# SaeedRahmani/MPC_for_AV_at_Intersection

Hardware: AMD Instinct MI355X
Metric: MPC timesteps/sec (whole node), N=20 horizon, 8-agent intersection, batch=4096 (higher is better)
Workload: dtype f64

## Files before the change

### mpc_for_av_at_intersection_amd/csrc/mpcx_common.h

```cpp
#pragma once
#include <hip/hip_runtime.h>
#include <stdint.h>
#include "mpcx.h"
#include "mpcx_qp_consts.h"
#include <vector>

struct mpcx_ctx {
    int device = 0;
    hipStream_t stream = nullptr;
    mpcx_mpc_params mpc = {};
    bool have_mpc = false;
    int32_t *ticket = nullptr;
    int n_cu = 0;
    double *pred = nullptr;
    size_t pred_cap = 0;
    hipGraphExec_t loop_exec = nullptr;
    unsigned char loop_key[1192] = {};
    const mpcx_qp_tuning *tune = nullptr;
    int32_t tune_rows = 0;
    const int32_t *order_hint = nullptr;
    const int32_t *order_now = nullptr, *order_prev = nullptr;
    int32_t *prev_cut = nullptr;
    size_t prev_cut_cap = 0;
    int32_t *order = nullptr;
    size_t order_cap = 0;
    int32_t *bins = nullptr;
    size_t bins_cap = 0;
    bool bins_clean = false;
    hipStream_t side = nullptr;
    hipEvent_t ev_fork = nullptr, ev_join = nullptr;
    double *cs = nullptr;
    size_t cs_cap = 0;
    void *multi = nullptr;
    size_t multi_cap = 0;
    int qp_solver = 0;
    int lin_passes = 1;
    bool prof_qp = false;
    std::vector<hipEvent_t> prof_ev;
    std::vector<hipEvent_t> prof_free;
    unsigned long long *stats = nullptr;
    size_t stats_slots = 0;
    void *comm = nullptr;
    int comm_world = 1, comm_rank = 0;
    double *xchg = nullptr;
    size_t xchg_cap = 0;
    double *admit_tab = nullptr;
    size_t admit_tab_cap = 0;
    char err[256] = {};
};

struct mpcx_interaction_extras {
    const double *pack_state = nullptr, *pack_applied = nullptr;
    const int32_t *ego_row = nullptr, *actor_row = nullptr;
    int32_t n_ego = 0, n_actors = 0;
    int32_t *prev_save = nullptr;
    const int32_t *key_prev = nullptr;
    int32_t *near = nullptr;
    const int32_t *bin_hint = nullptr;
    const int32_t *done = nullptr;
    const int32_t *absent = nullptr;
    const int32_t *prec = nullptr;
    double *stand = nullptr;
};
struct mpcx_window_extras {
    bool scatter = false;
    const int32_t *near = nullptr, *tidx = nullptr;
    bool rollout_forked = false;
    const int32_t *stop_idx = nullptr;
    double v_ref = 0.0;
    int32_t *len_seen = nullptr;
    const int32_t *done = nullptr;
    int32_t *queue_len = nullptr;
};
struct mpcx_qp_order {
    bool ready = false;
    const int32_t *hint = nullptr, *now = nullptr, *prev = nullptr;
    const int32_t *queue_len = nullptr;
};
struct mpcx_plant_extras {
    const int32_t *stats_iters = nullptr;
    bool reset_bins = false;
    const int32_t *done = nullptr;
};
int32_t mpcx_interaction_enqueue(mpcx_ctx *ctx, const mpcx_interaction_params *ip, int32_t P, const double *state, const double *path_xyyaw,
                               const double *path_cs, const int32_t *path_off, const int32_t *path_len, const int32_t *prev_cut_len,
                               int32_t n_obs_pool, const double *obs6, const int32_t *obs_off, const int32_t *obs_cnt, const int32_t *obs_skip,
                               int32_t *traj_idx, int32_t *hit_idx, double *hit_xy, int32_t *cut_len, const mpcx_interaction_extras &x);
int32_t mpcx_window_enqueue(mpcx_ctx *ctx, int32_t B, const double *state, const double *u_warm, const double *path_xyyaw, const double *path_v,
                          const int32_t *path_off, const int32_t *path_len, double dl, int32_t *target_ind, const double *ov, int64_t ov_stride,
                          double *xref, uint8_t *reaches_end, double *xbar, const mpcx_window_extras &x);
int32_t mpcx_qp_enqueue(mpcx_ctx *ctx, int32_t B, const double *x0, const double *xref, const double *xbar, const uint8_t *reaches_end,
                      const double *u_warm, double *x_out, double *u_out, int32_t *status, int32_t *iters, double *kkt, const mpcx_qp_order &ord);
int32_t mpcx_plant_enqueue(mpcx_ctx *ctx, int32_t B, double *state, double *u, const int32_t *status, double *applied, const mpcx_plant_extras &x);

int32_t mpcx_fail(mpcx_ctx *ctx, int32_t code, const char *fmt, ...);
int32_t mpcx_check_launch(mpcx_ctx *ctx, const char *what);
int32_t mpcx_grow(mpcx_ctx *ctx, void **p, size_t *cap_bytes, size_t need_bytes, const char *what);
int32_t mpcx_ensure_pred(mpcx_ctx *ctx, size_t need_doubles);
int32_t mpcx_rollout_fork(mpcx_ctx *ctx, int32_t B, const double *state, const double *u_warm, double *xbar, const int32_t *done = nullptr);
int32_t mpcx_traffic_validate(mpcx_ctx *ctx, int32_t n_actors, const mpcx_traffic_actor *actors, const double *tape, int64_t tape_rows,
                              const int32_t *pool_row, int32_t n_obs_pool);
int32_t mpcx_traffic_enqueue(mpcx_ctx *ctx, int32_t n_actors, const mpcx_traffic_actor *actors, double *actor_state, const double *tape,
                             int64_t tape_rows, const int32_t *pool_row, int32_t n_obs_pool, double *obs6);
bool mpcx_record_absent(const mpcx_run_log *log);
int32_t mpcx_record_validate(mpcx_ctx *ctx, const mpcx_run_log *log, const int32_t *obs_skip);
int32_t mpcx_record_enqueue(mpcx_ctx *ctx, const mpcx_interaction_params *ip, int32_t P, const double *state, const double *applied,
                            const double *x_sol, const double *path_xyyaw, const int32_t *path_off, const int32_t *path_len,
                            const int32_t *target_ind, const int32_t *cut_len, const int32_t *traj_idx, const int32_t *hit_idx,
                            const int32_t *status, const int32_t *iters, int32_t n_obs_pool, const double *obs6, const int32_t *obs_off,
                            const int32_t *obs_cnt, const int32_t *obs_skip, const mpcx_run_log *log,
                            const int32_t *goal_len = nullptr,
                            const int32_t *done = nullptr,
                            const int32_t *absent = nullptr);
bool mpcx_retire_absent(const mpcx_retire *r);
int32_t mpcx_retire_validate(mpcx_ctx *ctx, const mpcx_retire *r, int32_t P);
int32_t mpcx_retire_enqueue(mpcx_ctx *ctx, int32_t P, const double *state, double *applied, const double *path_xyyaw, const int32_t *path_off,
                            const int32_t *path_len, const int32_t *target_ind, const int32_t *goal_len, const mpcx_retire *r,
                            const mpcx_scene *scene = nullptr, const int32_t *own_row = nullptr);
bool mpcx_scene_absent(const mpcx_scene *s);
int32_t mpcx_scene_validate(mpcx_ctx *ctx, const mpcx_scene *s, const mpcx_retire *retire, int32_t exchange, size_t pool_rows, const int32_t *obs_skip);
bool mpcx_admit_absent(const mpcx_admit *a);
int32_t mpcx_admit_validate(mpcx_ctx *ctx, const mpcx_admit *a, const mpcx_retire *retire, const mpcx_scene *scene, int32_t exchange);
int32_t mpcx_admit_prepare(mpcx_ctx *ctx, size_t n_rows);
int32_t mpcx_admit_enqueue(mpcx_ctx *ctx, const mpcx_interaction_params *ip, int32_t P, const double *state, const int32_t *obs_off,
                           const int32_t *obs_cnt, const int32_t *obs_skip, int32_t *done, int32_t n_obs_pool, int32_t *absent,
                           int32_t n_actors, const mpcx_traffic_actor *actors, const double *actor_state, const double *tape,
                           int64_t tape_rows, const int32_t *actor_row, const mpcx_admit *admit);
bool mpcx_respawn_absent(const mpcx_respawn *s);
int32_t mpcx_respawn_validate(mpcx_ctx *ctx, const mpcx_respawn *s, const mpcx_admit *admit);
int32_t mpcx_respawn_enqueue(mpcx_ctx *ctx, int32_t P, double *state, double *applied, double *u_sol, int32_t *traj_idx, int32_t *target_ind,
                             int32_t *cut_len, int32_t *iters, int32_t *prev_len , const int32_t *obs_skip, int32_t n_obs_pool,
                             const mpcx_run_log *log , const mpcx_retire *retire, const mpcx_admit *admit,
                             const mpcx_respawn *respawn);
bool mpcx_routes_absent(const mpcx_routes *s);
int32_t mpcx_routes_validate(mpcx_ctx *ctx, const mpcx_routes *s, const mpcx_respawn *respawn, const int32_t *path_off, const int32_t *path_len,
                             int32_t max_len );
int32_t mpcx_route_enqueue(mpcx_ctx *ctx, int32_t P, double *state, double *applied, double *u_sol, int32_t *traj_idx, int32_t *target_ind,
                           int32_t *cut_len, int32_t *iters, int32_t *prev_len , const int32_t *obs_skip, int32_t n_obs_pool,
                           const mpcx_run_log *log , const mpcx_retire *retire, const mpcx_admit *admit,
                           const mpcx_respawn *respawn, const mpcx_routes *routes);
bool mpcx_precedence_absent(const mpcx_precedence *s);
int32_t mpcx_precedence_validate(mpcx_ctx *ctx, const mpcx_precedence *s, const mpcx_scene *scene, const mpcx_admit *admit);
int32_t mpcx_precedence_enqueue(mpcx_ctx *ctx, int32_t P, const int32_t *obs_off, const int32_t *obs_skip, const mpcx_admit *admit,
                                const mpcx_precedence *precedence);
bool mpcx_signals_absent(const mpcx_signals *s);
int32_t mpcx_signals_validate(mpcx_ctx *ctx, const mpcx_signals *s, int32_t exchange);
int32_t mpcx_signal_enqueue(mpcx_ctx *ctx, int32_t P, double dl, const double *state, const int32_t *path_off, const int32_t *path_len,
                            const int32_t *traj_idx, int32_t *cut_len, const int32_t *done , const mpcx_signals *signals);
int32_t mpcx_ensure_ticket(mpcx_ctx *ctx);
#define MPCX_JUMP_BONUS 11
#define MPCX_ORDER_BINS 64
#define MPCX_TICKET_WORDS 8
#define MPCX_TICKET_QUEUE_LEN 6
#define MPCX_ORDER_COPIES 16
namespace mpcx {
__device__ __forceinline__ int order_key_of(int hint, bool moved) {
    int k = hint < 0 ? 0 : hint;
    if (moved) k += MPCX_JUMP_BONUS;
    return k < MPCX_ORDER_BINS ? k : MPCX_ORDER_BINS - 1;
}
}
int32_t mpcx_ensure_order(mpcx_ctx *ctx, size_t B);
int32_t mpcx_qp_build_order(mpcx_ctx *ctx, int32_t B, const int32_t *hint, const int32_t *now, const int32_t *prev, hipStream_t st);

namespace mpcx {

constexpr int WAVE = 64;

struct QpArgs {
    mpcx_mpc_params p;
    int B;
    int32_t *ticket;
    int has_warm;
    const double *x0, *xref, *xbar, *u_warm;
    const uint8_t *re;
    double *x_out, *u_out, *kkt;
    int32_t *status, *iters;
    const mpcx_qp_tuning *tune;
    int has_tune;
    const int32_t *order;
    int has_order;
    int defer_fail;
    int32_t *fail_list, *fail_count;
    const int32_t *queue_len;
    int has_queue_len;
};

void launch_qp_stage(const QpArgs &a, hipStream_t st, int n_cu);
int qp_stage_grid(int B, int n_cu);

__device__ __forceinline__ double rdlane(double v, int l) {
    int lo = __double2loint(v), hi = __double2hiint(v);
    lo = __builtin_amdgcn_readlane(lo, l);
    hi = __builtin_amdgcn_readlane(hi, l);
    return __hiloint2double(hi, lo);
}
__device__ __forceinline__ double frcp(double d) {
    double r = __builtin_amdgcn_rcp(d);
    r = fma(fma(-d, r, 1.0), r, r);
    r = fma(fma(-d, r, 1.0), r, r);
    return r;
}

template <int CTRL, int ROW_MASK = 0xF>
__device__ __forceinline__ double dpp_mov(double old, double src) {
    int lo = __builtin_amdgcn_update_dpp(__double2loint(old), __double2loint(src), CTRL, ROW_MASK, 0xF, false);
    int hi = __builtin_amdgcn_update_dpp(__double2hiint(old), __double2hiint(src), CTRL, ROW_MASK, 0xF, false);
    return __hiloint2double(hi, lo);
}
__device__ __forceinline__ double lane_next(double v, double fill = 0.0) { return dpp_mov<0x130>(fill, v); }
__device__ __forceinline__ double lane_prev(double v, double fill = 0.0) { return dpp_mov<0x138>(fill, v); }

__device__ __forceinline__ double scan_up32(double v) {
    v += dpp_mov<0x111>(0.0, v);
    v += dpp_mov<0x112>(0.0, v);
    v += dpp_mov<0x114>(0.0, v);
    v += dpp_mov<0x118>(0.0, v);
    v += dpp_mov<0x142, 0xA>(0.0, v);
    return v;
}
__device__ __forceinline__ double scan_down32(double v, int lane) {
    v += dpp_mov<0x101>(0.0, v);
    v += dpp_mov<0x102>(0.0, v);
    v += dpp_mov<0x104>(0.0, v);
    v += dpp_mov<0x108>(0.0, v);
    const double r1 = rdlane(v, 16);
    return v + ((lane < 16) ? r1 : 0.0);
}
__device__ __forceinline__ double wave_sum_dpp(double v) {
    v += dpp_mov<0x111>(0.0, v);
    v += dpp_mov<0x112>(0.0, v);
    v += dpp_mov<0x114>(0.0, v);
    v += dpp_mov<0x118>(0.0, v);
    return (rdlane(v, 15) + rdlane(v, 31)) + (rdlane(v, 47) + rdlane(v, 63));
}
__device__ __forceinline__ double wave_max_dpp(double v) {
    v = fmax(v, dpp_mov<0x111>(v, v));
    v = fmax(v, dpp_mov<0x112>(v, v));
    v = fmax(v, dpp_mov<0x114>(v, v));
    v = fmax(v, dpp_mov<0x118>(v, v));
    return fmax(fmax(rdlane(v, 15), rdlane(v, 31)), fmax(rdlane(v, 47), rdlane(v, 63)));
}
__device__ __forceinline__ double frcp1(double d) {
    double r = __builtin_amdgcn_rcp(d);
    return fma(fma(-d, r, 1.0), r, r);
}

__device__ __forceinline__ void wave_argmin(double &d, int &i) {
#pragma unroll
    for (int s = 32; s >= 1; s >>= 1) {
        double od = __shfl_xor(d, s, WAVE);
        int oi = __shfl_xor(i, s, WAVE);
        bool take = (od < d) || (od == d && oi < i);
        d = take ? od : d;
        i = take ? oi : i;
    }
}

template <typename T>
__device__ __forceinline__ T wave_min_i(T v) {
#pragma unroll
    for (int s = 32; s >= 1; s >>= 1) { T o = __shfl_xor(v, s, WAVE); v = o < v ? o : v; }
    return v;
}

__device__ __forceinline__ void disc_centre(double px, double py, double c, double s, double cx, double cy, double &ex, double &ey) {
    ex = __dadd_rn(__dadd_rn(__dmul_rn(c, cx), -__dmul_rn(s, cy)), px);
    ey = __dadd_rn(__dadd_rn(__dmul_rn(s, cx), __dmul_rn(c, cy)), py);
}

struct Top3 {
    double d0 = INFINITY, d1 = INFINITY, d2 = INFINITY, s2 = INFINITY, s1 = INFINITY, s0 = INFINITY;
    int i0 = 0x7fffffff, i1 = 0x7fffffff, i2 = 0x7fffffff;
    __device__ __forceinline__ void offer(double px, double py, double x, double y, int i) {
        const double dx = __dadd_rn(px, -x), dy = __dadd_rn(py, -y);
        const double q = __dadd_rn(__dmul_rn(dx, dx), __dmul_rn(dy, dy));
        if (q < s2 || i2 == 0x7fffffff) {
            const double d = __dsqrt_rn(q);
            if (d < d2 || (d == d2 && i < i2)) {
                if (d < d1 || (d == d1 && i < i1)) {
                    d2 = d1; i2 = i1; s2 = s1;
                    if (d < d0 || (d == d0 && i < i0)) { d1 = d0; i1 = i0; s1 = s0; d0 = d; i0 = i; s0 = q; }
                    else { d1 = d; i1 = i; s1 = q; }
                } else { d2 = d; i2 = i; s2 = q; }
            }
        }
    }
    __device__ __forceinline__ void pop3(int (&bi)[3]) {
#pragma unroll
        for (int r = 0; r < 3; r++) {
            double d = d0; int ix = i0;
            wave_argmin(d, ix);
            bi[r] = ix;
            if (i0 == ix) { d0 = d1; i0 = i1; d1 = d2; i1 = i2; d2 = INFINITY; i2 = 0x7fffffff; }
        }
    }
};
__device__ __forceinline__ int three_nearest(const int (&bi)[3], int base) {
    if (abs(bi[1] - bi[2]) == 2) return bi[0] + base;
    if (abs(bi[0] - bi[1]) == 1) return max(bi[0], bi[1]) + base;
    return -1;
}

__device__ inline int nearest_index_in_direction(const double *path, int n, int start, double x, double y, int lane) {
    const int len = n - start;
    if (len <= 1) return start;
    if (len == 2) return start + 1;
    Top3 top;
    constexpr int DEPTH = 4;
    double bx[DEPTH], by[DEPTH];
#pragma unroll
    for (int k = 0; k < DEPTH; k++) {
        const int i = k * WAVE + lane;
        const double *q = path + 3 * (size_t)(start + (i < len ? i : 0));
        const double vx = q[0], vy = q[1];
        bx[k] = vx; by[k] = vy;
    }
    for (int i0 = 0; i0 < len; i0 += DEPTH * WAVE) {
        double nbx[DEPTH], nby[DEPTH];
#pragma unroll
        for (int k = 0; k < DEPTH; k++) {
            const int i = i0 + (DEPTH + k) * WAVE + lane;
            const double *q = path + 3 * (size_t)(start + (i < len ? i : 0));
            nbx[k] = q[0]; nby[k] = q[1];
        }
#pragma unroll
        for (int k = 0; k < DEPTH; k++) {
            const int i = i0 + k * WAVE + lane;
            if (i < len) top.offer(bx[k], by[k], x, y, i);
        }
#pragma unroll
        for (int k = 0; k < DEPTH; k++) { bx[k] = nbx[k]; by[k] = nby[k]; }
    }
    int bi[3];
#pragma unroll
    for (int r = 0; r < 3; r++) {
        double d = top.d0; int ix = top.i0;
        wave_argmin(d, ix);
        bi[r] = ix;
        if (top.i0 == ix) { top.d0 = top.d1; top.i0 = top.i1; top.d1 = top.d2; top.i1 = top.i2; top.d2 = INFINITY; top.i2 = 0x7fffffff; }
    }
    return three_nearest(bi, start);
}

}
```

### mpc_for_av_at_intersection_amd/csrc/mpcx_qp_quad.hip

```cpp
#include "mpcx_common.h"
#include "mpcx_qp_stage.h"

namespace mpcx {

typedef __attribute__((address_space(3))) double lds_double;

template <int LQ_, int SPL_, bool JERK_ = false>
struct GroupCx {
    static constexpr int LQ = LQ_, SPL = SPL_;
    static constexpr bool JERK = JERK_;
    static_assert(LQ == 8, "groups of 8 lanes");
    int q, lane;
    lds_double *sh;
    __device__ __forceinline__ double nxt(double v) const { return dpp_mov<0x101>(v, v); }
    __device__ __forceinline__ double prv(double v) const { return dpp_mov<0x111>(v, v); }
    __device__ __forceinline__ double gsum(double v) const {
        v += dpp_mov<0xB1>(v, v); v += dpp_mov<0x4E>(v, v);
        v += dpp_mov<0x141>(v, v);
        return v;
    }
    __device__ __forceinline__ double gmax(double v) const {
        v = fmax(v, dpp_mov<0xB1>(v, v)); v = fmax(v, dpp_mov<0x4E>(v, v));
        v = fmax(v, dpp_mov<0x141>(v, v));
        return v;
    }
    __device__ __forceinline__ double gmin(double v) const {
        v = fmin(v, dpp_mov<0xB1>(v, v)); v = fmin(v, dpp_mov<0x4E>(v, v));
        v = fmin(v, dpp_mov<0x141>(v, v));
        return v;
    }
    __device__ __forceinline__ bool gany(bool b) const {
        const unsigned long long m = __ballot(b);
        return ((m >> (lane & ~(LQ - 1))) & ((1ull << LQ) - 1ull)) != 0ull;
    }
    __device__ __forceinline__ bool any(bool b) const { return __ballot(b) != 0ull; }
    __device__ __forceinline__ int count(bool b) const { return __popcll(__ballot(b)); }
    __device__ __forceinline__ double rcp(double v) const { return frcp(v); }
    __device__ __forceinline__ double rcp_fast(double v) const { return frcp1(v); }
    __device__ __forceinline__ double rcp_seed(double v) const { return __builtin_amdgcn_rcp(v); }
    __device__ __forceinline__ void fence() const { asm volatile("" ::: "memory"); }
    __device__ __forceinline__ void stamp(int) const {}
    __device__ __forceinline__ double ld_s(int k) const { return sh[(0 * SPL * 8 + k) * 64 + lane]; }
    __device__ __forceinline__ double ld_l(int k) const { return sh[(1 * SPL * 8 + k) * 64 + lane]; }
    __device__ __forceinline__ double ld_k(int k) const { return sh[(2 * SPL * 8 + k) * 64 + lane]; }
    __device__ __forceinline__ void st_s(int k, double v) { sh[(0 * SPL * 8 + k) * 64 + lane] = v; }
    __device__ __forceinline__ void st_l(int k, double v) { sh[(1 * SPL * 8 + k) * 64 + lane] = v; }
    __device__ __forceinline__ void st_k(int k, double v) { sh[(2 * SPL * 8 + k) * 64 + lane] = v; }
    __device__ __forceinline__ double ld_w(int k) const { return sh[(3 * SPL * 8 + k) * 64 + lane]; }
    __device__ __forceinline__ void st_w(int k, double v) { sh[(3 * SPL * 8 + k) * 64 + lane] = v; }
};

constexpr int REFILL_GROUPS = 2;
template <int LQ, int SPL, bool TUNED>
struct QueueSrc {
    const QpArgs &a;
    __device__ __forceinline__ mpcx_mpc_params params() const { return a.p; }
    __device__ __forceinline__ mpcx_stage::Problem at(int b) const {
        const int T = a.p.T, W = T + 1;
        return mpcx_stage::Problem{a.x0 + (size_t)b * 4, a.xref + (size_t)b * 4 * W, a.xbar + (size_t)b * 4 * W,
                                   a.has_warm ? a.u_warm + (size_t)b * 2 * T : nullptr, a.re + (size_t)b * W,
                                   a.x_out + (size_t)b * 4 * W, a.u_out + (size_t)b * 2 * T, a.kkt + (size_t)b * 4,
                                   a.status + b, a.iters + b};
    }
    __device__ __forceinline__ int refill_min() const { return REFILL_GROUPS * LQ; }
    __device__ __forceinline__ long max_rounds() const { return ((long)a.B + 2) * (long)(a.p.max_iter + 6) * (MPCX_POLISH_TRIES + 1); }
    template <class Cx>
    __device__ __forceinline__ bool fetch(Cx &cx, mpcx_mpc_params &P, int &pbi) const {
        int t = 0;
        if (cx.q == 0) t = atomicAdd(a.ticket, 1);
        t = (int)cx.gsum((double)t);
        const bool have = t < (a.has_queue_len ? *a.queue_len : a.B);
        const int b = have ? (a.has_order ? a.order[t] : t) : 0;
        pbi = b;
        if (TUNED) {
            const mpcx_qp_tuning &tu = a.tune[b];
            P.w_perp = tu.w_perp; P.w_para = tu.w_para;
            P.R[0] = tu.R[0]; P.R[1] = tu.R[1]; P.Rd[0] = tu.Rd[0]; P.Rd[1] = tu.Rd[1];
            P.Q_v_yaw[0] = tu.Q_v_yaw[0]; P.Q_v_yaw[1] = tu.Q_v_yaw[1];
            P.Qf[0] = tu.Qf[0]; P.Qf[1] = tu.Qf[1]; P.Qf[2] = tu.Qf[2]; P.Qf[3] = tu.Qf[3];
            P.max_accel = tu.max_accel; P.max_decel = tu.max_decel; P.max_dsteer = tu.max_dsteer;
        }
        return have;
    }
};

template <int LQ, int SPL, bool TUNED, bool JERK>
__global__ __launch_bounds__(64, 1) void qp_quad_kernel(QpArgs a) {
    if (a.has_queue_len && *a.queue_len == 0) return;
    __shared__ double sh[(3 * SPL * 8 + 2 * SPL) * 64];
    const int lane = threadIdx.x;
    GroupCx<LQ, SPL, JERK> cx{lane & (LQ - 1), lane, (lds_double *)sh};
    QueueSrc<LQ, SPL, TUNED> src{a};
    mpcx_stage::solve_queue(cx, src);
}

int qp_stage_grid(int B, int n_cu) {
    const int need = (B + 7) / 8;
    const int resident = n_cu * 4;
    return need < resident ? need : resident;
}

template <int LQ, int SPL, bool JERK>
void launch_qp_group(const QpArgs &a, hipStream_t st, int n_cu) {
    static_assert(LQ == 8, "qp_stage_grid counts eight lane groups per wavefront");
    const int grid = qp_stage_grid(a.B, n_cu);
    if (a.has_tune) hipLaunchKernelGGL((qp_quad_kernel<LQ, SPL, true, JERK>), dim3(grid), dim3(64), 0, st, a);
    else hipLaunchKernelGGL((qp_quad_kernel<LQ, SPL, false, JERK>), dim3(grid), dim3(64), 0, st, a);
}

void launch_qp_stage(const QpArgs &a, hipStream_t st, int n_cu) {
    const int T = a.p.T;
    if (a.p.model == MPCX_MODEL_JERK5) {
        if (T <= 16) launch_qp_group<8, 2, true>(a, st, n_cu);
        else if (T <= 24) launch_qp_group<8, 3, true>(a, st, n_cu);
        else launch_qp_group<8, 4, true>(a, st, n_cu);
        return;
    }
    if (T <= 16) launch_qp_group<8, 2, false>(a, st, n_cu);
    else if (T <= 24) launch_qp_group<8, 3, false>(a, st, n_cu);
    else launch_qp_group<8, 4, false>(a, st, n_cu);
}

}
```

Baseline: 8.768 million.

## Pack nine seven-lane QP groups per wavefront when horizon fits

Adds a seven-lane group context so that, when ceil(T/SPL) is at most 7 (as with T=20, SPL=3), a 64-lane wavefront runs nine QP problems instead of eight, leaving lane 63 idle. Group reductions use row-shift DPP chains plus a ds_bpermute broadcast from the group base lane, because seven-lane groups do not line up with DPP row boundaries. Grid sizing is changed to take the group width into account. The exchange is more expensive reductions (extra shifts and an LDS-path permute) for about 12% more problems per wave, and the nxt/prv neighbour semantics change across group edges.

Result: no change. 8.692 million (-0.9%).

```diff
diff --git a/mpc_for_av_at_intersection_amd/csrc/mpcx_common.h b/mpc_for_av_at_intersection_amd/csrc/mpcx_common.h
--- a/mpc_for_av_at_intersection_amd/csrc/mpcx_common.h
+++ b/mpc_for_av_at_intersection_amd/csrc/mpcx_common.h
@@ -187,7 +187,7 @@
 };
 
 void launch_qp_stage(const QpArgs &a, hipStream_t st, int n_cu);
-int qp_stage_grid(int B, int n_cu);
+int qp_stage_grid(int B, int n_cu, int lanes_per_group);
 
 __device__ __forceinline__ double rdlane(double v, int l) {
     int lo = __double2loint(v), hi = __double2hiint(v);
@@ -210,6 +210,11 @@
 }
 __device__ __forceinline__ double lane_next(double v, double fill = 0.0) { return dpp_mov<0x130>(fill, v); }
 __device__ __forceinline__ double lane_prev(double v, double fill = 0.0) { return dpp_mov<0x138>(fill, v); }
+__device__ __forceinline__ double lane_fetch(int addr4, double v) {
+    const int lo = __builtin_amdgcn_ds_bpermute(addr4, __double2loint(v));
+    const int hi = __builtin_amdgcn_ds_bpermute(addr4, __double2hiint(v));
+    return __hiloint2double(hi, lo);
+}
 
 __device__ __forceinline__ double scan_up32(double v) {
     v += dpp_mov<0x111>(0.0, v);
diff --git a/mpc_for_av_at_intersection_amd/csrc/mpcx_qp_quad.hip b/mpc_for_av_at_intersection_amd/csrc/mpcx_qp_quad.hip
--- a/mpc_for_av_at_intersection_amd/csrc/mpcx_qp_quad.hip
+++ b/mpc_for_av_at_intersection_amd/csrc/mpcx_qp_quad.hip
@@ -33,6 +33,61 @@
         const unsigned long long m = __ballot(b);
         return ((m >> (lane & ~(LQ - 1))) & ((1ull << LQ) - 1ull)) != 0ull;
     }
+    __device__ __forceinline__ bool leader() const { return q == 0; }
+    __device__ __forceinline__ bool live() const { return true; }
+    __device__ __forceinline__ bool any(bool b) const { return __ballot(b) != 0ull; }
+    __device__ __forceinline__ int count(bool b) const { return __popcll(__ballot(b)); }
+    __device__ __forceinline__ double rcp(double v) const { return frcp(v); }
+    __device__ __forceinline__ double rcp_fast(double v) const { return frcp1(v); }
+    __device__ __forceinline__ double rcp_seed(double v) const { return __builtin_amdgcn_rcp(v); }
+    __device__ __forceinline__ void fence() const { asm volatile("" ::: "memory"); }
+    __device__ __forceinline__ void stamp(int) const {}
+    __device__ __forceinline__ double ld_s(int k) const { return sh[(0 * SPL * 8 + k) * 64 + lane]; }
+    __device__ __forceinline__ double ld_l(int k) const { return sh[(1 * SPL * 8 + k) * 64 + lane]; }
+    __device__ __forceinline__ double ld_k(int k) const { return sh[(2 * SPL * 8 + k) * 64 + lane]; }
+    __device__ __forceinline__ void st_s(int k, double v) { sh[(0 * SPL * 8 + k) * 64 + lane] = v; }
+    __device__ __forceinline__ void st_l(int k, double v) { sh[(1 * SPL * 8 + k) * 64 + lane] = v; }
+    __device__ __forceinline__ void st_k(int k, double v) { sh[(2 * SPL * 8 + k) * 64 + lane] = v; }
+    __device__ __forceinline__ double ld_w(int k) const { return sh[(3 * SPL * 8 + k) * 64 + lane]; }
+    __device__ __forceinline__ void st_w(int k, double v) { sh[(3 * SPL * 8 + k) * 64 + lane] = v; }
+};
+
+template <int SPL_, bool JERK_ = false>
+struct GroupCx7 {
+    static constexpr int LQ = 7, SPL = SPL_;
+    static constexpr bool JERK = JERK_;
+    int q, lane;
+    lds_double *sh;
+    __device__ __forceinline__ double nxt(double v) const { return dpp_mov<0x130>(v, v); }
+    __device__ __forceinline__ double prv(double v) const { return dpp_mov<0x138>(v, v); }
+    __device__ __forceinline__ double gsum(double v) const {
+        const double o = nxt(v);
+        const double s = v + (q == 6 ? 0.0 : o);
+        const double t = s + nxt(nxt(s));
+        const int base = 4 * (lane - q);
+        const double w = t + nxt(nxt(nxt(nxt(t))));
+        return lane_fetch(base, w);
+    }
+    __device__ __forceinline__ double gmax(double v) const {
+        v = fmax(v, nxt(v));
+        v = fmax(v, nxt(nxt(v)));
+        const int base = 4 * (lane - q);
+        v = fmax(v, nxt(nxt(nxt(v))));
+        return lane_fetch(base, v);
+    }
+    __device__ __forceinline__ double gmin(double v) const {
+        v = fmin(v, nxt(v));
+        v = fmin(v, nxt(nxt(v)));
+        const int base = 4 * (lane - q);
+        v = fmin(v, nxt(nxt(nxt(v))));
+        return lane_fetch(base, v);
+    }
+    __device__ __forceinline__ bool gany(bool b) const {
+        const unsigned long long m = __ballot(b);
+        return ((m >> (lane - q)) & 0x7full) != 0ull;
+    }
+    __device__ __forceinline__ bool leader() const { return q == 0 && lane < 63; }
+    __device__ __forceinline__ bool live() const { return lane < 63; }
     __device__ __forceinline__ bool any(bool b) const { return __ballot(b) != 0ull; }
     __device__ __forceinline__ int count(bool b) const { return __popcll(__ballot(b)); }
     __device__ __forceinline__ double rcp(double v) const { return frcp(v); }
@@ -67,9 +122,9 @@
     template <class Cx>
     __device__ __forceinline__ bool fetch(Cx &cx, mpcx_mpc_params &P, int &pbi) const {
         int t = 0;
-        if (cx.q == 0) t = atomicAdd(a.ticket, 1);
+        if (cx.leader()) t = atomicAdd(a.ticket, 1);
         t = (int)cx.gsum((double)t);
-        const bool have = t < (a.has_queue_len ? *a.queue_len : a.B);
+        const bool have = cx.live() && t < (a.has_queue_len ? *a.queue_len : a.B);
         const int b = have ? (a.has_order ? a.order[t] : t) : 0;
         pbi = b;
         if (TUNED) {
@@ -89,36 +144,48 @@
     if (a.has_queue_len && *a.queue_len == 0) return;
     __shared__ double sh[(3 * SPL * 8 + 2 * SPL) * 64];
     const int lane = threadIdx.x;
-    GroupCx<LQ, SPL, JERK> cx{lane & (LQ - 1), lane, (lds_double *)sh};
     QueueSrc<LQ, SPL, TUNED> src{a};
-    mpcx_stage::solve_queue(cx, src);
+    if constexpr (LQ == 7) {
+        GroupCx7<SPL, JERK> cx{lane % 7, lane, (lds_double *)sh};
+        mpcx_stage::solve_queue(cx, src);
+    } else {
+        GroupCx<LQ, SPL, JERK> cx{lane & (LQ - 1), lane, (lds_double *)sh};
+        mpcx_stage::solve_queue(cx, src);
+    }
 }
 
-int qp_stage_grid(int B, int n_cu) {
-    const int need = (B + 7) / 8;
+int qp_stage_grid(int B, int n_cu, int lanes_per_group) {
+    const int groups = 64 / lanes_per_group;
+    const int need = (B + groups - 1) / groups;
     const int resident = n_cu * 4;
     return need < resident ? need : resident;
 }
 
 template <int LQ, int SPL, bool JERK>
 void launch_qp_group(const QpArgs &a, hipStream_t st, int n_cu) {
-    static_assert(LQ == 8, "qp_stage_grid counts eight lane groups per wavefront");
-    const int grid = qp_stage_grid(a.B, n_cu);
+    static_assert(LQ == 8 || LQ == 7, "groups of eight or seven lanes");
+    const int grid = qp_stage_grid(a.B, n_cu, LQ);
     if (a.has_tune) hipLaunchKernelGGL((qp_quad_kernel<LQ, SPL, true, JERK>), dim3(grid), dim3(64), 0, st, a);
     else hipLaunchKernelGGL((qp_quad_kernel<LQ, SPL, false, JERK>), dim3(grid), dim3(64), 0, st, a);
+}
+
+template <int SPL, bool JERK>
+void launch_qp_spl(const QpArgs &a, hipStream_t st, int n_cu) {
+    if ((a.p.T + SPL - 1) / SPL <= 7) launch_qp_group<7, SPL, JERK>(a, st, n_cu);
+    else launch_qp_group<8, SPL, JERK>(a, st, n_cu);
 }
 
 void launch_qp_stage(const QpArgs &a, hipStream_t st, int n_cu) {
     const int T = a.p.T;
     if (a.p.model == MPCX_MODEL_JERK5) {
-        if (T <= 16) launch_qp_group<8, 2, true>(a, st, n_cu);
-        else if (T <= 24) launch_qp_group<8, 3, true>(a, st, n_cu);
-        else launch_qp_group<8, 4, true>(a, st, n_cu);
+        if (T <= 16) launch_qp_spl<2, true>(a, st, n_cu);
+        else if (T <= 24) launch_qp_spl<3, true>(a, st, n_cu);
+        else launch_qp_spl<4, true>(a, st, n_cu);
         return;
     }
-    if (T <= 16) launch_qp_group<8, 2, false>(a, st, n_cu);
-    else if (T <= 24) launch_qp_group<8, 3, false>(a, st, n_cu);
-    else launch_qp_group<8, 4, false>(a, st, n_cu);
+    if (T <= 16) launch_qp_spl<2, false>(a, st, n_cu);
+    else if (T <= 24) launch_qp_spl<3, false>(a, st, n_cu);
+    else launch_qp_spl<4, false>(a, st, n_cu);
 }
 
 }
```
